# davidegraff/notorch

Measured on AMD Instinct MI355X. Metric: edge-messages/sec D-MPNN depth=3 h=300, QM9-shaped batches, 1/2/4/8 MI355X, higher is better.
Workload: dtype f32; 1 GPU; qm9-4096: 4096 qm9-shaped molecules per GPU, D-MPNN depth=3 hidden=300, ChempropBlock + Sum readout, reference collate (rev offset by nodes); molecules_per_gpu=4096, V_per_gpu=36362, E_per_gpu=77562, hidden=300, depth=3, parallelism=molecule-sharded x1, no collective on the forward path

## Files before the change

notorch_amd/csrc/update_fk.hip:

```cpp
#include <stdlib.h>

#include <atomic>

#include <type_traits>

#include "common.hpp"
#include "update.hpp"

#include "update_fk.hpp"

namespace nt {
int cu_count();
int xcd_count();
}

namespace nt {
namespace {
template <int RT, int CT, int ACT, int AACT, bool SUMONLY, int MAXL, bool DROP = false>
int launch_fk_t(const fk::Args& a, int grid, hipStream_t stream) {
  if constexpr (DROP)
    set_last_kernel(RT == 8 ? "update_fk_kernel: one 8-wave workgroup per CU, 128-row tiles, dropout in the epilogue"
                            : "update_fk_kernel: one 8-wave workgroup per CU, 64-row tiles, dropout in the epilogue");
  else
    set_last_kernel(RT == 8 ? "update_fk_kernel: one 8-wave workgroup per CU, 128-row tiles"
                            : "update_fk_kernel: one 8-wave workgroup per CU, 64-row tiles");
  fk::update_fk_kernel<RT, CT, ACT, AACT, SUMONLY, MAXL, 0, 8, DROP><<<grid, fk::kThreads, 0, stream>>>(a);
  NT_LAUNCH_CHECK();
  return NT_OK;
}

template <int CT, bool DROP = false>
int launch_fk_wide(const fk::Args& a, int maxl, int grid, hipStream_t stream) {
  [[maybe_unused]] const bool fused = a.SO != nullptr;
  const bool relu = a.act == NT_ACT_RELU;
  if constexpr (!DROP) {
    if (!fused) {
      if (relu) return launch_fk_t<8, CT, NT_ACT_RELU, NT_ACT_IDENTITY, true, 1>(a, grid, stream);
      if (a.act == NT_ACT_IDENTITY)
        return launch_fk_t<8, CT, NT_ACT_IDENTITY, NT_ACT_IDENTITY, true, 1>(a, grid, stream);
      return launch_fk_t<8, CT, -1, NT_ACT_IDENTITY, true, 1>(a, grid, stream);
    }
  }
  if (a.aact == NT_ACT_RELU)
    return maxl <= 3   ? launch_fk_t<8, CT, NT_ACT_RELU, NT_ACT_RELU, true, 3, DROP>(a, grid, stream)
           : maxl <= 8 ? launch_fk_t<8, CT, NT_ACT_RELU, NT_ACT_RELU, true, 8, DROP>(a, grid, stream)
                       : launch_fk_t<8, CT, NT_ACT_RELU, NT_ACT_RELU, true, 16, DROP>(a, grid, stream);
  return maxl <= 3   ? launch_fk_t<8, CT, NT_ACT_RELU, NT_ACT_IDENTITY, true, 3, DROP>(a, grid, stream)
         : maxl <= 8 ? launch_fk_t<8, CT, NT_ACT_RELU, NT_ACT_IDENTITY, true, 8, DROP>(a, grid, stream)
                     : launch_fk_t<8, CT, NT_ACT_RELU, NT_ACT_IDENTITY, true, 16, DROP>(a, grid, stream);
}

int fk_nw_env() {
  static const int v = [] {
    const char* e = getenv("NT_FK_NW");
    return e ? atoi(e) : 0;
  }();
  return v;
}
bool fk_nw4(int64_t h, bool fused, int act, int reduce, int aact) {
  return fk_nw_env() != 8 && fused && act == NT_ACT_RELU && reduce == NT_SUM &&
         (aact == NT_ACT_RELU || aact == NT_ACT_IDENTITY) && fk::nt_for(h) <= 20;
}
bool fk_nw4_forced() { return fk_nw_env() == 4; }

template <int AACT, int MAXL, bool DROP>
int launch_fk_nw4_t(const fk::Args& a, int grid, hipStream_t stream) {
  set_last_kernel(DROP ? "update_fk_kernel: two 4-wave workgroups per CU, 64-row tiles, dropout in the epilogue"
                       : "update_fk_kernel: two 4-wave workgroups per CU, 64-row tiles");
  fk::update_fk_kernel<4, 5, NT_ACT_RELU, AACT, true, MAXL, 0, 4, DROP><<<grid, 256, 0, stream>>>(a);
  NT_LAUNCH_CHECK();
  return NT_OK;
}

template <bool DROP = false>
int launch_fk_nw4(const fk::Args& a, int maxl, int grid, hipStream_t stream) {
  if (a.aact == NT_ACT_RELU)
    return maxl <= 3   ? launch_fk_nw4_t<NT_ACT_RELU, 3, DROP>(a, grid, stream)
           : maxl <= 8 ? launch_fk_nw4_t<NT_ACT_RELU, 8, DROP>(a, grid, stream)
                       : launch_fk_nw4_t<NT_ACT_RELU, 16, DROP>(a, grid, stream);
  return maxl <= 3   ? launch_fk_nw4_t<NT_ACT_IDENTITY, 3, DROP>(a, grid, stream)
         : maxl <= 8 ? launch_fk_nw4_t<NT_ACT_IDENTITY, 8, DROP>(a, grid, stream)
                     : launch_fk_nw4_t<NT_ACT_IDENTITY, 16, DROP>(a, grid, stream);
}

template <int CT, bool DROP = false>
int launch_fk_narrow(const fk::Args& a, int maxl, int grid, hipStream_t stream) {
  const bool fused = a.SO != nullptr;
  const bool relu = a.act == NT_ACT_RELU;
  const bool fast = !fused || (a.reduce == NT_SUM && (a.aact == NT_ACT_RELU || a.aact == NT_ACT_IDENTITY));
  if (fast) {
    if constexpr (!DROP) {
      if (!fused)
        return relu ? launch_fk_t<4, CT, NT_ACT_RELU, NT_ACT_IDENTITY, true, 1>(a, grid, stream)
                    : launch_fk_t<4, CT, -1, NT_ACT_IDENTITY, true, 1>(a, grid, stream);
    }
    if (a.aact == NT_ACT_RELU)
      return relu ? launch_fk_t<4, CT, NT_ACT_RELU, NT_ACT_RELU, true, 16, DROP>(a, grid, stream)
                  : launch_fk_t<4, CT, -1, NT_ACT_RELU, true, 16, DROP>(a, grid, stream);
    return relu ? launch_fk_t<4, CT, NT_ACT_RELU, NT_ACT_IDENTITY, true, 16, DROP>(a, grid, stream)
                : launch_fk_t<4, CT, -1, NT_ACT_IDENTITY, true, 16, DROP>(a, grid, stream);
  }
  (void)maxl;
  return launch_fk_t<4, CT, -1, -1, false, 16, DROP>(a, grid, stream);
}
}

int fk_tile_rows(int64_t h, int act, int reduce, int aact, bool fused) {
  if (fk_nw4_forced() && fk_nw4(h, fused, act, reduce, aact)) return 64;
  const bool wide_ok =
      !fused || (act == NT_ACT_RELU && reduce == NT_SUM && (aact == NT_ACT_RELU || aact == NT_ACT_IDENTITY));
  return (fk::nt_for(h) <= 24 && wide_ok) ? 128 : 64;
}

int launch_update_fk(const UpdateArgs& u, const void* Wimg, const float* amax_in, float* amax_out,
                     const int32_t* tile_ptr, int64_t ntiles, int tile_rows, int max_in_degree,
                     const void* row_table, int reduce, int aact, float aalpha, float* S_out,
                     const DropMask* drop) {
  const bool fused = tile_ptr != nullptr;
  NT_REQUIRE(fused == (S_out != nullptr), NT_EINVAL, "S_out must be given exactly with a tile plan");
  NT_REQUIRE(!fused || row_table, NT_EINVAL, "fp32 fused mode needs the row table (nt_dmpnn_row_table)");
  NT_REQUIRE(drop == nullptr || fused, NT_EUNSUPPORTED, "the dropout layer kernel needs a tile plan");
  NT_REQUIRE(amax_in != nullptr, NT_EINVAL, "fp32 update needs amax_in (max|H|, max|S| on the device)");
  NT_REQUIRE(u.h % 4 == 0, NT_EUNSUPPORTED, "fp32 update needs h % 4 == 0");
  NT_REQUIRE((u.E * u.h) / 4 < (int64_t(1) << 31) && (u.V * u.h) / 4 < (int64_t(1) << 31),
             NT_EUNSUPPORTED, "fp32 update: E*h and V*h must stay below 2^33");
  const int cap = fk_tile_rows(u.h, u.act, reduce, aact, fused);
  NT_REQUIRE(!fused || (tile_rows >= 1 && tile_rows <= cap), NT_EUNSUPPORTED,
             "tile plan rows exceed nt_dmpnn_fused_tile_rows for this layer");
  NT_REQUIRE(!fused || (max_in_degree >= 0 && max_in_degree <= 32), NT_EUNSUPPORTED,
             "fused aggregation needs max_in_degree <= 32");
  fk::Args a;
  a.H = u.H;
  a.S = u.S;
  a.src = u.src;
  a.rev = u.rev;
  a.Wimg = (const char*)Wimg;
  a.bias = u.b;
  a.amax_in = amax_in;
  a.amax_out = amax_out;
  a.V = u.V;
  a.E = u.E;
  a.h = (int)u.h;
  a.hv = (int)(u.h / 4);
  {
    const int64_t ldi = u.ldi ? u.ldi : u.h, ldo = u.ldo ? u.ldo : u.h;
    NT_REQUIRE(ldi >= u.h && ldo >= u.h && ldi % 4 == 0 && ldo % 4 == 0, NT_EINVAL,
               "row pitches must be >= h and multiples of 4");
    NT_REQUIRE((u.E * ldi) / 4 < (int64_t(1) << 31) && (u.V * ldi) / 4 < (int64_t(1) << 31) &&
                   (u.E * ldo) / 4 < (int64_t(1) << 31) && (u.V * ldo) / 4 < (int64_t(1) << 31),
               NT_EUNSUPPORTED, "fp32 update: E*ld and V*ld must stay below 2^33");
    a.ldiv = a.ldic = (int)(ldi / 4);
    a.ldoc = (int)(ldo / 4);
  }
  a.KS = fk::ks_for(u.h) < 4 ? 4 : (fk::ks_for(u.h) + 1) / 2 * 2;
  a.NT = fk::nt_for(u.h);
  a.residual = u.residual;
  a.act = u.act;
  a.alpha = u.alpha;
  a.tile_ptr = tile_ptr;
  a.rows = fused ? (const int4*)row_table : nullptr;
  a.reduce = reduce;
  a.aact = aact;
  a.aalpha = aalpha;
  a.O = u.H_out;
  a.SO = S_out;
  a.SP = u.S_part;
  if (drop) a.drop = *drop;
  a.nxcd = xcd_count();
  {
    static const int stagger = [] {
      const char* e = getenv("NT_FK_STAGGER");
      return e ? atoi(e) : 0;
    }();
    a.stagger = stagger;
  }
  a.ntiles = fused ? (int)ntiles : (int)((u.E + cap - 1) / cap);
  if (a.ntiles == 0) return NT_OK;
  const int grid = a.ntiles < cu_count() ? a.ntiles : cu_count();
  const int maxl = max_in_degree - 1;
  if (fused && tile_rows <= 64 && fk_nw4(u.h, true, u.act, reduce, aact)) {
    a.nchunks = 1;
    const int g4 = a.ntiles < 2 * cu_count() ? a.ntiles : 2 * cu_count();
    return drop ? launch_fk_nw4<true>(a, maxl, g4, u.stream) : launch_fk_nw4(a, maxl, g4, u.stream);
  }
  if (cap == 128) {
    a.nchunks = 1;
    return drop ? launch_fk_wide<3, true>(a, maxl, grid, u.stream) : launch_fk_wide<3>(a, maxl, grid, u.stream);
  }
  if (a.NT <= 24) {
    a.nchunks = 1;
    return drop ? launch_fk_narrow<3, true>(a, maxl, grid, u.stream) : launch_fk_narrow<3>(a, maxl, grid, u.stream);
  }
  a.nchunks = (a.NT + 31) / 32;
  return drop ? launch_fk_narrow<4, true>(a, maxl, grid, u.stream) : launch_fk_narrow<4>(a, maxl, grid, u.stream);
}

namespace {
template <int ACT, int AACT, bool SUMONLY, int MAXL>
int launch_fkb_t(const fk::Args& a, int grid, hipStream_t stream) {
  set_last_kernel("update_fk_kernel (bf16): one 8-wave workgroup per CU, 128-row tiles");
  fk::update_fk_kernel<8, 4, ACT, AACT, SUMONLY, MAXL, 1><<<grid, fk::kThreads, 0, stream>>>(a);
  NT_LAUNCH_CHECK();
  return NT_OK;
}
template <int AACT, int MAXL>
// ... 145 lines not shown
```

notorch_amd/csrc/update_fk.hpp:

```cpp
#pragma once

#include <type_traits>

#include "common.hpp"
#include "dropout.hpp"

namespace nt {
namespace fk {

typedef float f32x4 __attribute__((ext_vector_type(4)));
typedef _Float16 f16x8 __attribute__((ext_vector_type(8)));
typedef _Float16 f16x4 __attribute__((ext_vector_type(4)));
typedef __bf16 bf16x8 __attribute__((ext_vector_type(8)));
typedef __bf16 bf16x4 __attribute__((ext_vector_type(4)));

__device__ __forceinline__ float bf_lo(unsigned u) { return __uint_as_float(u << 16); }
__device__ __forceinline__ float bf_hi(unsigned u) { return __uint_as_float(u & 0xffff0000u); }
__device__ __forceinline__ float4 bf4_widen(uint4 v) {
  return float4{bf_lo(v.x), bf_hi(v.x), bf_lo(v.y), bf_hi(v.y)};
}
__device__ __forceinline__ uint2 bf4_pack(float a, float b, float c, float d) {
  const bf16x4 v = bf16x4{(__bf16)a, (__bf16)b, (__bf16)c, (__bf16)d};
  return __builtin_bit_cast(uint2, v);
}

constexpr int kThreads = 512;
constexpr int kWaves = 8;
constexpr int kImgHdr = 256;
constexpr int kEmaps = 4;
constexpr int kFlagStart = 1, kFlagEnd = 2, kFlagPart = 4;

__host__ __device__ constexpr int ks_for(int64_t h) { return (int)((h + 31) / 32); }
__host__ __device__ constexpr int nt_for(int64_t h) { return (int)((h + 15) / 16); }
__host__ __device__ constexpr int64_t image_bytes(int64_t h) {
  return kImgHdr + (int64_t)ks_for(h) * nt_for(h) * 2 * 1024;
}

struct Args {
  const float* H;
  const float* S;
  const int64_t* src;
  const int64_t* rev;
  const char* Wimg;
  const float* bias;
  const float* amax_in;
  float* amax_out;
  int64_t V, E;
  int h, hv, KS, NT, nchunks;
  int ldiv, ldic, ldoc;
  int residual, act;
  float alpha;
  const int* tile_ptr;
  int ntiles;
  const int4* rows;
  int reduce, aact;
  float aalpha;
  float* O;
  float* SO;
  float* SP = nullptr;
  int nxcd;
  int stagger;
  DropMask drop;
};

__host__ __device__ inline int scale_exp(float bound) {
  if (!(bound > 0.f) || !(bound <= 3.4028235e38f)) return 0;
  int e;
  frexpf(bound, &e);
  int s = 14 - e;
  return s > 24 ? 24 : s;
}

__device__ __forceinline__ float act_bound(float m, int act, float alpha) {
  if (act == NT_ACT_RELU || act == NT_ACT_IDENTITY) return m;
  const float a = fabsf(alpha) > 1.f ? fabsf(alpha) : 1.f;
  return a * m + a;
}

__device__ __forceinline__ void atomic_max_abs(float* p, float v) {
  atomic_max_nonneg(p, v);
}

__device__ __forceinline__ float wave_max(float v) {
#pragma unroll
  for (int o = 32; o >= 1; o >>= 1) v = fmaxf(v, __shfl_xor(v, o));
  return v;
}

__device__ __forceinline__ f16x8 as_f16x8(uint4 v) { return __builtin_bit_cast(f16x8, v); }

constexpr float kLoScale = 2048.f;
__device__ __forceinline__ _Float16 lo_part(float x, _Float16 x0) { return (_Float16)((x - (float)x0) * kLoScale); }

template <typename F, int... Is>
__device__ __forceinline__ void sfor_impl(F&& f, std::integer_sequence<int, Is...>) {
  (f(std::integral_constant<int, Is>{}), ...);
}
template <int N, typename F>
__device__ __forceinline__ void sfor(F&& f) {
  sfor_impl(f, std::make_integer_sequence<int, N>{});
}

__device__ __forceinline__ float dpp_shr1(float old, float x) {
  return __builtin_bit_cast(float, __builtin_amdgcn_update_dpp(__builtin_bit_cast(int, old),
                                                               __builtin_bit_cast(int, x), 0x111, 0xf,
                                                               0xf, false));
}
__device__ __forceinline__ float dpp_shr1_bc(float x) {
  return __builtin_bit_cast(float, __builtin_amdgcn_mov_dpp(__builtin_bit_cast(int, x), 0x111, 0xf, 0xf, true));
}
__device__ __forceinline__ float dpp_ror1(float x) {
  return __builtin_bit_cast(float, __builtin_amdgcn_update_dpp(0, __builtin_bit_cast(int, x), 0x121,
                                                               0xf, 0xf, false));
}

struct TileHead {
  int T, n;
};

template <int RT, bool PLAN>
__device__ __forceinline__ TileHead tile_head(const Args& a, int t) {
  if constexpr (PLAN) {
    const int T = a.tile_ptr[t], n = a.tile_ptr[t + 1] - T;
    return {T, n};
  }
  const int64_t T = (int64_t)t * (16 * RT);
  const int64_t n = a.E - T < 16 * RT ? a.E - T : 16 * RT;
  return {(int)T, (int)n};
}

template <int RT, bool FROM_ROWS>
__device__ __forceinline__ int4 row_raw(const Args& a, TileHead th, int row) {
  const int pos = th.T + (row < th.n ? row : 0);
  if constexpr (FROM_ROWS) return a.rows[pos];
  const int s = a.src ? (int)a.src[pos] : pos;
  const int q = a.rev ? (int)a.rev[pos] : -1;
  return int4{pos, s, q, kFlagStart | kFlagEnd};
}

__device__ __forceinline__ int2 row_offsets(const Args& a, int4 raw, bool valid) {
  const bool sok = valid && raw.y >= 0 && raw.y < a.V, qok = valid && raw.z >= 0 && raw.z < a.E;
  return int2{sok ? raw.y * a.ldiv : -1, qok ? raw.z * a.ldiv : -1};
}

__device__ __forceinline__ int4 row_entry(int4 raw, bool valid) {
  if (!valid) return int4{-1, -1, kFlagStart | kFlagEnd, 0};
  if (raw.w >= 0) return int4{raw.x, raw.w >> 2, raw.w & 3, 0};
  const int wv = -raw.w - 1;
  return int4{raw.x, wv >> 2, (wv & 3) | kFlagPart, 0};
}

constexpr int kGD = 2;

template <int RT, int CT, int PREC = 0, int NW = 8>
struct State {
  static constexpr int ROWS = 16 * RT;
  static constexpr int PPT = 2 * RT / NW;
  static constexpr int kPartB = RT * 1024;
  static constexpr int kBufB = 2 * kPartB;
  f32x4 acc[RT][CT];
  f32x4 bias[CT];
  uint4 wb[2][CT][2];
  f32x4 gs[kGD][PPT], gq[kGD][PPT];
  int gso[kGD], gqo[kGD];
  float mxH, mxS;
  int lane, wave, fr, g16, grt, grow, kp0, hv, hc, NT, CTC;
  int li, lo;
  float sA, sAW, inv;
  char* abuf;
  float* lbias;
  int4* emap;
  __amdgpu_buffer_rsrc_t wrsrc;
};

template <int RT, int CT, int ACT, int P, int PREC, int NW>
__device__ __forceinline__ void fk_gather(State<RT, CT, PREC, NW>& st, const Args& a, int soff, int qoff, int s) {
  st.gso[P] = soff;
  st.gqo[P] = qoff;
  const int sb = soff >= 0 ? soff : 0, qb = qoff >= 0 ? qoff : 0;
  const f32x4* S4 = reinterpret_cast<const f32x4*>(a.S);
  const f32x4* H4 = reinterpret_cast<const f32x4*>(a.H ? a.H : a.S);
  constexpr int NP = PREC ? 1 : State<RT, CT, PREC, NW>::PPT;
#pragma unroll
  for (int u = 0; u < NP; ++u) {
    int p = PREC ? 4 * s + st.g16 : 8 * s + st.kp0 + u;
    p = p < st.hv ? p : 0;
    st.gs[P][u] = S4[sb + p];
    st.gq[P][u] = H4[qb + p];
  }
}

template <int RT, int CT, int ACT, int P, int BUF, int PREC, int NW>
__device__ __forceinline__ void fk_split(State<RT, CT, PREC, NW>& st, const Args& a, int s) {
  using St = State<RT, CT, PREC, NW>;
  const bool sok = st.gso[P] >= 0, qok = st.gqo[P] >= 0;
  if constexpr (PREC == 1) {
    static_assert(RT == NW, "bf16 fk tiles: one row tile per wave");
    const bool in = 4 * s + st.g16 < st.hv;
    const uint4 su = __builtin_bit_cast(uint4, st.gs[P][0]), qu = __builtin_bit_cast(uint4, st.gq[P][0]);
    const unsigned sw[4] = {su.x, su.y, su.z, su.w}, qw[4] = {qu.x, qu.y, qu.z, qu.w};
    bf16x8 h0;
#pragma unroll
    for (int c = 0; c < 4; ++c) {
      const float q0 = act_t<ACT>(bf_lo(qw[c]), a.act, a.alpha), q1 = act_t<ACT>(bf_hi(qw[c]), a.act, a.alpha);
      h0[2 * c] = (__bf16)((sok && in ? bf_lo(sw[c]) : 0.f) - (qok && in ? q0 : 0.f));
      h0[2 * c + 1] = (__bf16)((sok && in ? bf_hi(sw[c]) : 0.f) - (qok && in ? q1 : 0.f));
    }
    *reinterpret_cast<bf16x8*>(st.abuf + BUF * St::kBufB + st.grt * 1024 + st.lane * 16) = h0;
    return;
  }
  float x[4 * St::PPT];
#pragma unroll
  for (int u = 0; u < St::PPT; ++u) {
    const bool in = 8 * s + st.kp0 + u < st.hv;
    const f32x4 sv = st.gs[P][u];
    const f32x4 qv = st.gq[P][u];
#pragma unroll
    for (int c = 0; c < 4; ++c) {
      const float q = act_t<ACT>(qv[c], a.act, a.alpha);
      const float av = (sok && in ? sv[c] : 0.f) - (qok && in ? q : 0.f);
      x[4 * u + c] = av * st.sA;
    }
  }
  char* base = st.abuf + BUF * St::kBufB + st.grt * 1024 + st.lane * 16 +
               (RT == NW ? 0 : 8 * (st.wave >> 2));
// ... 35 lines not shown
  }
}

__device__ __forceinline__ f16x8 w0_lo_scaled(uint4 w) {
  const unsigned k = 0x10001000u;
  uint4 r;
  asm volatile("v_pk_mul_f16 %0, %1, %2" : "=v"(r.x) : "v"(w.x), "s"(k));
  asm volatile("v_pk_mul_f16 %0, %1, %2" : "=v"(r.y) : "v"(w.y), "s"(k));
  asm volatile("v_pk_mul_f16 %0, %1, %2" : "=v"(r.z) : "v"(w.z), "s"(k));
  asm volatile("v_pk_mul_f16 %0, %1, %2" : "=v"(r.w) : "v"(w.w), "s"(k));
  return as_f16x8(r);
}

template <int PREC>
__device__ __forceinline__ f32x4 fk_mac(uint4 w0r, uint4 w1r, f16x8 a0, f16x8 a1, f32x4 t) {
  if constexpr (PREC == 1) {
    return __builtin_amdgcn_mfma_f32_16x16x32_bf16(__builtin_bit_cast(bf16x8, w0r), __builtin_bit_cast(bf16x8, a0),
                                                   t, 0, 0, 0);
  } else {
    const f16x8 w0 = as_f16x8(w0r), w1 = as_f16x8(w1r);
    t = __builtin_amdgcn_mfma_f32_16x16x32_f16(w1, a0, t, 0, 0, 0);
    t = __builtin_amdgcn_mfma_f32_16x16x32_f16(w0_lo_scaled(w0r), a1, t, 0, 0, 0);
    return __builtin_amdgcn_mfma_f32_16x16x32_f16(w0, a0, t, 0, 0, 0);
  }
}

template <int RT, int CT, int P, int PREC, int NW>
__device__ __forceinline__ void fk_mfma(State<RT, CT, PREC, NW>& st, int c, int nrt) {
  using St = State<RT, CT, PREC, NW>;
  const char* bb = st.abuf + P * St::kBufB + st.lane * 16;
  f16x8 a0 = *reinterpret_cast<const f16x8*>(bb);
  f16x8 a1 = PREC ? a0 : *reinterpret_cast<const f16x8*>(bb + St::kPartB);
#pragma unroll
  for (int rt = 0; rt < RT; ++rt) {
    if (rt < nrt) {
      f16x8 n0 = a0, n1 = a1;
      if (rt + 1 < RT) {
        n0 = *reinterpret_cast<const f16x8*>(bb + (rt + 1) * 1024);
        n1 = PREC ? n0 : *reinterpret_cast<const f16x8*>(bb + St::kPartB + (rt + 1) * 1024);
      }
#pragma unroll
      for (int j = 0; j < CT; ++j) {
        if (c * st.CTC + st.wave + NW * j < st.NT) {
          st.acc[rt][j] = fk_mac<PREC>(st.wb[P][j][0], st.wb[P][j][1], a0, a1, st.acc[rt][j]);
        }
      }
      a0 = n0;
      a1 = n1;
      __builtin_amdgcn_sched_barrier(0);
    }
  }
}

template <int RT, int CT, int PREC, int NW>
__device__ __forceinline__ void fk_resid_load(State<RT, CT, PREC, NW>& st, const Args& a, int i, int c, int j) {
  using St = State<RT, CT, PREC, NW>;
  int pc = 4 * (c * st.CTC + st.wave + NW * j) + st.g16;
  pc = pc < st.hc ? pc : 0;
#pragma unroll
  for (int rt = 0; rt < RT; ++rt) {
    const int e = st.emap[(i % kEmaps) * St::ROWS + 16 * rt + st.fr].x;
    const int64_t r = (int64_t)(e >= 0 ? e : 0) * st.li + pc;
    if constexpr (PREC == 1) {
      const uint2 v = reinterpret_cast<const uint2*>(a.H)[r];
      st.acc[rt][j] = __builtin_bit_cast(f32x4, uint4{v.x, v.y, 0u, 0u});
    } else {
      st.acc[rt][j] = reinterpret_cast<const f32x4*>(a.H)[r];
    }
  }
}

template <int RT, int CT, int PREC, int NW>
__device__ __forceinline__ void fk_bias_load(State<RT, CT, PREC, NW>& st, const Args& a, int c, int j) {
  int pc = 4 * (c * st.CTC + st.wave + NW * j) + st.g16;
  pc = (pc < st.hc && a.bias) ? pc : 0;
  if constexpr (PREC == 1) {
    const uint2 v = reinterpret_cast<const uint2*>(a.bias ? a.bias : a.S)[pc];
    st.bias[j] = __builtin_bit_cast(f32x4, uint4{v.x, v.y, 0u, 0u});
  } else {
    st.bias[j] = reinterpret_cast<const f32x4*>(a.bias ? a.bias : a.S)[pc];
  }
}

template <int RT, int CT, int PREC, int NW>
__device__ __forceinline__ void fk_resid_scale(State<RT, CT, PREC, NW>& st) {
  if constexpr (PREC == 1) {
#pragma unroll
    for (int rt = 0; rt < RT; ++rt)
#pragma unroll
      for (int j = 0; j < CT; ++j) {
        const float4 w = bf4_widen(__builtin_bit_cast(uint4, st.acc[rt][j]));
        st.acc[rt][j] = f32x4{w.x, w.y, w.z, w.w};
      }
    return;
  }
  const f32x4 s4 = f32x4{st.sAW, st.sAW, st.sAW, st.sAW};
#pragma unroll
  for (int rt = 0; rt < RT; ++rt)
#pragma unroll
    for (int j = 0; j < CT; ++j) st.acc[rt][j] = st.acc[rt][j] * s4;
}

constexpr bool fk_lds_bias(int NW) { return NW == 4; }

struct EpiCtx {
  const f32x4* b4;
  f32x4* O4;
  f32x4* SO4;
  const int4* em;
  int n;
  const f32x4* H4 = nullptr;
};

template <int RTI, int J, int RT, int CT, int AACT, bool SUMONLY, int MAXL, bool DROP, int PREC, int NW>
__device__ __forceinline__ void fk_epi_row(State<RT, CT, PREC, NW>& st, const Args& a, const EpiCtx& x0, int pc,
                                           bool pok, const f32x4& bj, f32x4& carry, float& ccnt) {
  if (16 * RTI < x0.n) {
    const int lo = st.lo;
    const int4 ri = x0.em[16 * RTI + st.fr];
    f32x4 o;
    [[maybe_unused]] f32x4 hres = f32x4{0.f, 0.f, 0.f, 0.f};
    if constexpr (DROP) {
      if (x0.H4) hres = x0.H4[(int64_t)(ri.x >= 0 ? ri.x : 0) * st.li + (pok ? pc : 0)];
    }
    uint2 ob = uint2{0u, 0u};
    if constexpr (PREC == 1) {
      ob = bf4_pack(st.acc[RTI][J][0] + bj[0], st.acc[RTI][J][1] + bj[1], st.acc[RTI][J][2] + bj[2],
                    st.acc[RTI][J][3] + bj[3]);
      const float4 w = bf4_widen(uint4{ob.x, ob.y, 0u, 0u});
      o = f32x4{w.x, w.y, w.z, w.w};
    } else {
#pragma unroll
      for (int q = 0; q < 4; ++q) o[q] = fmaf(st.acc[RTI][J][q], st.inv, bj[q]);
      if constexpr (DROP) {
        const uint64_t i0 = (uint64_t)(ri.x >= 0 ? ri.x : 0) * (uint64_t)a.h + (uint64_t)(4 * pc);
#pragma unroll
        for (int q = 0; q < 4; ++q) o[q] = hres[q] + drop_apply(a.drop, i0 + q, o[q]);
      }
    }
    const bool rok = ri.x >= 0 && pok;
    if (rok) {
      if constexpr (PREC == 1) {
        reinterpret_cast<uint2*>(x0.O4)[(int64_t)ri.x * lo + pc] = ob;
      } else {
        x0.O4[(int64_t)ri.x * lo + pc] = o;
        st.mxH = fmaxf(st.mxH, fmaxf(fmaxf(fabsf(o[0]), fabsf(o[1])), fmaxf(fabsf(o[2]), fabsf(o[3]))));
      }
    }
    if (x0.SO4 != nullptr) {
      const bool start = (ri.z & kFlagStart) != 0;
      f32x4 m;
#pragma unroll
      for (int q = 0; q < 4; ++q) m[q] = act_t<AACT>(o[q], a.aact, a.aalpha);
      f32x4 x = m, cin;
#pragma unroll
      for (int q = 0; q < 4; ++q) cin[q] = dpp_ror1(carry[q]);
      float cnt = 1.f;
      const float cinc = SUMONLY ? 0.f : dpp_ror1(ccnt);
#pragma unroll
      for (int it = 0; it < MAXL; ++it) {
        f32x4 y;
#pragma unroll
        for (int q = 0; q < 4; ++q) y[q] = dpp_shr1(cin[q], x[q]);
        if constexpr (SUMONLY) {
          x = start ? m : y + m;
        } else {
          const float yc = dpp_shr1(cinc, cnt);
          f32x4 z;
#pragma unroll
          for (int q = 0; q < 4; ++q) {
            const float mx = fmaxf(y[q], m[q]), mn = fminf(y[q], m[q]), sm = y[q] + m[q];
            z[q] = a.reduce == NT_MAX ? mx : (a.reduce == NT_MIN ? mn : sm);
          }
          x = start ? m : z;
          cnt = start ? 1.f : yc + 1.f;
        }
      }
      if ((ri.z & kFlagPart) && (ri.z & kFlagEnd) && rok) {
        if constexpr (PREC == 0) reinterpret_cast<f32x4*>(a.SP)[(int64_t)ri.y * st.hc + pc] = x;
      } else if ((ri.z & kFlagEnd) && rok) {
        f32x4 r = x;
        if (!SUMONLY && a.reduce == NT_MEAN) r = x / cnt;
        if constexpr (PREC == 1) {
          reinterpret_cast<uint2*>(x0.SO4)[(int64_t)ri.y * lo + pc] = bf4_pack(r[0], r[1], r[2], r[3]);
        } else {
          x0.SO4[(int64_t)ri.y * lo + pc] = r;
          st.mxS = fmaxf(st.mxS, fmaxf(fmaxf(fabsf(r[0]), fabsf(r[1])), fmaxf(fabsf(r[2]), fabsf(r[3]))));
        }
      }
      carry = x;
      ccnt = cnt;
    }
  }
  if constexpr (RTI + 1 < RT)
    fk_epi_row<RTI + 1, J, RT, CT, AACT, SUMONLY, MAXL, DROP>(st, a, x0, pc, pok, bj, carry, ccnt);
}

template <int J, int RT, int CT, int AACT, bool SUMONLY, int MAXL, bool DROP, int PREC, int NW>
__device__ __forceinline__ void fk_epi_col(State<RT, CT, PREC, NW>& st, const Args& a, const EpiCtx& x0, int i, int c,
                                           bool load_next, int i_next, int c_next) {
  const int ct = c * st.CTC + st.wave + NW * J;
  if (ct < st.NT) {
    const int pc = 4 * ct + st.g16;
    const bool pok = pc < st.hc;
    f32x4 bj = f32x4{0.f, 0.f, 0.f, 0.f};
    if constexpr (fk_lds_bias(NW)) {
      if (x0.b4 && pok) bj = *reinterpret_cast<const f32x4*>(st.lbias + 4 * pc);
    } else {
      if (x0.b4 && pok) bj = st.bias[J];
    }
    if constexpr (PREC == 1 && !fk_lds_bias(NW)) {
      const float4 w = bf4_widen(__builtin_bit_cast(uint4, bj));
      bj = f32x4{w.x, w.y, w.z, w.w};
    }
    f32x4 carry = f32x4{0.f, 0.f, 0.f, 0.f};
    float ccnt = 0.f;
    fk_epi_row<0, J, RT, CT, AACT, SUMONLY, MAXL, DROP>(st, a, x0, pc, pok, bj, carry, ccnt);
  }
  if (!fk_lds_bias(NW) && c_next != c) fk_bias_load(st, a, c_next, J);
  if (load_next) {
    fk_resid_load(st, a, i_next, c_next, J);
  } else {
#pragma unroll
    for (int rt = 0; rt < RT; ++rt) st.acc[rt][J] = f32x4{0.f, 0.f, 0.f, 0.f};
  }
  if constexpr (J + 1 < CT)
    fk_epi_col<J + 1, RT, CT, AACT, SUMONLY, MAXL, DROP>(st, a, x0, i, c, load_next, i_next, c_next);
}

template <int RT, int CT, int AACT, bool SUMONLY, int MAXL, bool DROP, int PREC, int NW>
__device__ __forceinline__ void fk_epilogue(State<RT, CT, PREC, NW>& st, const Args& a, int i, int c, int n,
                                            bool load_next, int i_next, int c_next) {
  EpiCtx x0;
  x0.b4 = reinterpret_cast<const f32x4*>(a.bias);
  x0.O4 = reinterpret_cast<f32x4*>(a.O);
  x0.SO4 = reinterpret_cast<f32x4*>(a.SO);
  x0.em = st.emap + (i % kEmaps) * State<RT, CT, PREC, NW>::ROWS;
  x0.n = n;
  if constexpr (DROP) {
    x0.H4 = (a.residual && a.H != nullptr) ? reinterpret_cast<const f32x4*>(a.H) : nullptr;
  }
  fk_epi_col<0, RT, CT, AACT, SUMONLY, MAXL, DROP>(st, a, x0, i, c, load_next, i_next, c_next);
}

constexpr int kLbiasB = 512 * 4;

__device__ __forceinline__ void fk_barrier() {
  __syncthreads();
}

template <int RT, int CT, int ACT, int AACT, bool SUMONLY, int MAXL, int PREC = 0, int NW = 8,
          bool DROP = false>
__global__ void __launch_bounds__(64 * NW, 2) update_fk_kernel(Args a) {
  static_assert(!DROP || PREC == 0, "the dropout epilogue is fp32 only (bf16: update_bf16_kernel)");
  constexpr bool FROM_ROWS = MAXL > 1;
  using St = State<RT, CT, PREC, NW>;
  constexpr int ROWS = St::ROWS;
  constexpr int kEmapB = kEmaps * ROWS * 16;
  static_assert(RT == NW || (RT == 4 && NW == 8), "row tiles per wave mapping");
  constexpr bool LB = fk_lds_bias(NW);
  constexpr int kExtraB = LB ? kLbiasB : 0;
  __shared__ __attribute__((aligned(16))) uint4 smem[(2 * St::kBufB + kEmapB + kExtraB) / 16];

  int t0 = (int)blockIdx.x, tstride = (int)gridDim.x, ntl;
  const int nx = a.nxcd;
  if (nx > 1 && (int)gridDim.x % nx == 0) {
    const int x = (int)blockIdx.x % nx, chunk = (a.ntiles + nx - 1) / nx;
    const int lo = x * chunk, hi = min(a.ntiles, lo + chunk);
    t0 = lo + (int)blockIdx.x / nx;
    tstride = (int)gridDim.x / nx;
    ntl = hi > t0 ? (hi - t0 + tstride - 1) / tstride : 0;
  } else {
    ntl = (a.ntiles - t0 + tstride - 1) / tstride;
  }
  if (ntl <= 0) return;
  auto tile = [&](int i) __attribute__((always_inline)) { return t0 + (i < ntl ? i : ntl - 1) * tstride; };
  if constexpr (NW == 4) {
    for (int q = (int)blockIdx.x >= (int)gridDim.x / 2 ? a.stagger : 0; q > 0; --q) __builtin_amdgcn_s_sleep(127);
  } else {
    for (int q = a.stagger * (((int)blockIdx.x / (nx > 0 ? nx : 1)) & 3); q > 0; --q) __builtin_amdgcn_s_sleep(127);
  }

  St st;
  const int tid = threadIdx.x;
  st.lane = tid & 63;
  st.wave = __builtin_amdgcn_readfirstlane(tid >> 6);
  st.fr = st.lane & 15;
  st.g16 = st.lane >> 4;
  st.grt = RT == NW ? st.wave : (st.wave & 3);
  st.grow = 16 * st.grt + st.fr;
  st.kp0 = RT == NW ? 2 * st.g16 : 2 * st.g16 + (st.wave >> 2);
  st.hv = a.hv;
  st.hc = a.h / 4;
  st.li = a.ldic;
  st.lo = a.ldoc;
  st.NT = a.NT;
  st.CTC = NW * CT;
  st.abuf = reinterpret_cast<char*>(smem);
  st.emap = reinterpret_cast<int4*>(st.abuf + 2 * St::kBufB);
  st.lbias = reinterpret_cast<float*>(st.abuf + 2 * St::kBufB + kEmapB);

  if constexpr (LB) {
    for (int q = tid; q < a.h; q += 64 * NW) {
      float b = 0.f;
      if (a.bias) {
        if constexpr (PREC == 1) b = __uint_as_float((unsigned)reinterpret_cast<const unsigned short*>(a.bias)[q] << 16);
        else b = a.bias[q];
      }
      st.lbias[q] = b;
    }
  }
  st.wrsrc = __builtin_amdgcn_make_buffer_rsrc(
      (void*)a.Wimg, (short)0, PREC ? ks_for(a.h) * nt_for(a.h) * 1024 : (int)image_bytes(a.h), 0x00020000);
  st.mxH = 0.f;
  st.mxS = 0.f;
  if constexpr (PREC == 1) {
    st.sA = st.sAW = st.inv = 1.f;
  } else {
    const float bound = a.src ? a.amax_in[1] + (a.rev ? act_bound(a.amax_in[0], a.act, a.alpha) : 0.f)
                              : a.amax_in[1];
    st.sA = ldexpf(1.f, scale_exp(bound));
    const float sW = *reinterpret_cast<const float*>(a.Wimg);
    st.sAW = st.sA * sW;
    st.inv = 1.f / st.sAW;
  }
  const bool resid = !DROP && a.residual && a.H != nullptr;
  const bool info_writer = st.g16 == 0 && st.wave < RT;
  const int SPT = a.nchunks * a.KS;

  int2 cur, nxt;
  int n_cur, n_nxt;
  int4 raw2;
  TileHead h2, h3;
  {
    const TileHead h0 = tile_head<RT, FROM_ROWS>(a, tile(0));
    const int4 r0 = row_raw<RT, FROM_ROWS>(a, h0, st.grow);
    const TileHead h1 = tile_head<RT, FROM_ROWS>(a, tile(1));
    const int4 r1 = row_raw<RT, FROM_ROWS>(a, h1, st.grow);
    h2 = tile_head<RT, FROM_ROWS>(a, tile(2));
    raw2 = row_raw<RT, FROM_ROWS>(a, h2, st.grow);
    h3 = tile_head<RT, FROM_ROWS>(a, tile(3));
    const bool v0 = st.grow < h0.n, v1 = st.grow < h1.n;
    cur = row_offsets(a, r0, v0);
    nxt = row_offsets(a, r1, v1);
    if (info_writer) {
      st.emap[0 * ROWS + st.grow] = row_entry(r0, v0);
      st.emap[1 * ROWS + st.grow] = row_entry(r1, v1);
    }
    n_cur = h0.n < ROWS ? h0.n : ROWS;
    n_nxt = h1.n < ROWS ? h1.n : ROWS;
  }
#pragma unroll
  for (int r = 0; r < RT; ++r)
#pragma unroll
    for (int j = 0; j < CT; ++j) st.acc[r][j] = f32x4{0.f, 0.f, 0.f, 0.f};

  __syncthreads();
  if (resid) {
#pragma unroll
    for (int j = 0; j < CT; ++j) fk_resid_load(st, a, 0, 0, j);
  }
#pragma unroll
  for (int j = 0; j < CT; ++j)
    if constexpr (!LB) fk_bias_load(st, a, 0, j);
  auto kcs = [&](int kk, int& cc, int& ss) __attribute__((always_inline)) {
    cc = kk / a.KS;
    ss = kk - cc * a.KS;
  };
  {
    int c1, s1;
    kcs(1, c1, s1);
    fk_gather<RT, CT, ACT, 0>(st, a, cur.x, cur.y, 0);
    fk_gather<RT, CT, ACT, 1>(st, a, cur.x, cur.y, 1 % a.KS);
    fk_load_w<RT, CT, 0>(st, 0, 0);
    fk_load_w<RT, CT, 1>(st, c1, s1);
    fk_split<RT, CT, ACT, 0, 0>(st, a, 0);
    fk_gather<RT, CT, ACT, 0>(st, a, cur.x, cur.y, 2 % a.KS);
  }
  fk_barrier();

  int i = 0, c = 0;
  const int U = ntl * a.nchunks;
  for (int u = 0; u < U; ++u) {
    fk_resid_scale(st);
    const int nrt = (n_cur + 15) >> 4;
    const int kb = c * a.KS;
    for (int s0 = 0; s0 < a.KS; s0 += 2) {
#pragma unroll
      for (int P = 0; P < 2; ++P) {
        const int k = kb + s0 + P;
        auto phase_mfma = [&]() __attribute__((always_inline)) {
          if (P == 0) fk_mfma<RT, CT, 0>(st, c, nrt);
          else fk_mfma<RT, CT, 1>(st, c, nrt);
          {
            int c2, s2;
            kcs(k + 2 < SPT ? k + 2 : k + 2 - SPT, c2, s2);
            if (P == 0) fk_load_w<RT, CT, 0>(st, c2, s2);
            else fk_load_w<RT, CT, 1>(st, c2, s2);
          }
        };
        auto phase_split = [&]() __attribute__((always_inline)) {
          const int k1 = k + 1 < SPT ? k + 1 : k + 1 - SPT;
          const int s1 = k1 - (k1 / a.KS) * a.KS;
          if (P == 0) fk_split<RT, CT, ACT, 1, 1>(st, a, s1);
          else fk_split<RT, CT, ACT, 0, 0>(st, a, s1);
          const int k3 = k + 3;
          const int adv = k3 >= SPT ? 1 : 0;
          const int s3 = (k3 - adv * SPT) % a.KS;
          const int so = adv == 0 ? cur.x : nxt.x, qo = adv == 0 ? cur.y : nxt.y;
          if (P == 0) fk_gather<RT, CT, ACT, 1>(st, a, so, qo, s3);
          else fk_gather<RT, CT, ACT, 0>(st, a, so, qo, s3);
        };
        phase_mfma();
        phase_split();
        fk_barrier();
      }
    }
    const bool last_c = c + 1 == a.nchunks;
    const int i_next = last_c ? (i + 1 < ntl ? i + 1 : i) : i, c_next = last_c ? 0 : c + 1;
    fk_epilogue<RT, CT, AACT, SUMONLY, MAXL, DROP>(st, a, i, c, n_cur, resid, i_next, c_next);
    c = c_next;
    if (last_c) {
      ++i;
      cur = nxt;
      n_cur = n_nxt;
      const bool v2 = st.grow < h2.n;
      nxt = row_offsets(a, raw2, v2);
      if (info_writer) st.emap[((i + 1) % kEmaps) * ROWS + st.grow] = row_entry(raw2, v2);
      n_nxt = h2.n < ROWS ? h2.n : ROWS;
      h2 = h3;
      raw2 = row_raw<RT, FROM_ROWS>(a, h2, st.grow);
      h3 = tile_head<RT, FROM_ROWS>(a, tile(i + 3));
    }
  }
  if (a.amax_out) {
    const float mh = wave_max(st.mxH), ms = wave_max(st.mxS);
    __shared__ float amx[2][NW];
    if (st.lane == 0) {
      amx[0][st.wave] = mh;
      amx[1][st.wave] = ms;
    }
    __syncthreads();
    if (tid == 0) {
      float bh = amx[0][0], bs = amx[1][0];
#pragma unroll
      for (int w = 1; w < NW; ++w) {
        bh = fmaxf(bh, amx[0][w]);
        bs = fmaxf(bs, amx[1][w]);
      }
      atomic_max_abs(a.amax_out, bh);
      if (a.SO) atomic_max_abs(a.amax_out + 1, bs);
    }
  }
}

__global__ void __launch_bounds__(256) row_table_kernel(const int32_t* __restrict__ perm,
                                                        const int32_t* __restrict__ dsts,
                                                        const int64_t* __restrict__ src,
                                                        const int64_t* __restrict__ rev, int64_t V,
                                                        int64_t E, int4* __restrict__ out) {
  for (int64_t p = blockIdx.x * 256LL + threadIdx.x; p < E; p += (int64_t)gridDim.x * 256) {
    const int e = perm[p];
    const int64_t s = src[e], q = rev[e];
    const int v = dsts[p];
    const bool start = p == 0 || dsts[p - 1] != v, end = p + 1 == E || dsts[p + 1] != v;
    out[p] = int4{e, (s >= 0 && s < V) ? (int)s : -1, (q >= 0 && q < E) ? (int)q : -1,
                  (v << 2) | (start ? kFlagStart : 0) | (end ? kFlagEnd : 0)};
  }
}

constexpr int kScaleParts = 32;
__global__ void __launch_bounds__(256) pack_fk_scale_kernel(const float* __restrict__ W, int64_t h,
                                                            int64_t w_stride, int64_t img_stride,
                                                            char* __restrict__ img) {
  const float* Wl = W + blockIdx.y * w_stride;
  const int64_t n = h * h, per = (n + kScaleParts - 1) / kScaleParts;
  const int64_t lo = blockIdx.x * per, hi = lo + per < n ? lo + per : n;
  __shared__ float red[4];
  float m = 0.f;
  for (int64_t q = lo + threadIdx.x; q < hi; q += 256) m = fmaxf(m, fabsf(Wl[q]));
  m = wave_max(m);
  if ((threadIdx.x & 63) == 0) red[threadIdx.x >> 6] = m;
  __syncthreads();
  if (threadIdx.x == 0)
    reinterpret_cast<float*>(img + blockIdx.y * img_stride)[1 + blockIdx.x] =
        fmaxf(fmaxf(red[0], red[1]), fmaxf(red[2], red[3]));
}

__global__ void __launch_bounds__(256) pack_fk_kernel(const float* __restrict__ W, int64_t h, int KS,
                                                      int NT, int64_t w_stride, int64_t img_stride,
                                                      char* __restrict__ img) {
  const int layer = blockIdx.y;
  const float* Wl = W + layer * w_stride;
  char* out = img + layer * img_stride;
  float mw = 0.f;
#pragma unroll
  for (int i = 1; i <= kScaleParts; ++i) mw = fmaxf(mw, reinterpret_cast<const float*>(out)[i]);
  const float sW = ldexpf(1.f, scale_exp(mw));
  if (blockIdx.x == 0 && threadIdx.x == 0) *reinterpret_cast<float*>(out) = sW;
  const int64_t slots = (int64_t)KS * NT * 2 * 64;
  const int64_t q = blockIdx.x * 256LL + threadIdx.x;
  if (q >= slots) return;
  const int l = (int)(q & 63);
  const int64_t blk = q >> 6;
// ... 96 lines not shown
```

Measured before the change: 598.0 million edge-messages/s.

## Add 32-bit byte-offset epilogue with buffer resource residual loads and ballot masks

Adds a B32 epilogue path for fp32 sum-only kernels without dropout. The row map stores precomputed 32-bit byte offsets, residual loads go through a buffer resource, and start/end/hub flags become wave ballot bitmasks that drive the segmented scan and masked stores. The amax reduction switches to LDS atomics. The aim is to cut 64-bit address arithmetic, per-row flag decoding and VGPR pressure in the epilogue. A 64-bit fallback is chosen automatically for large tensors or via an env var, which adds a template variant and code complexity.

```diff
diff --git a/notorch_amd/csrc/update_fk.hip b/notorch_amd/csrc/update_fk.hip
--- a/notorch_amd/csrc/update_fk.hip
+++ b/notorch_amd/csrc/update_fk.hip
@@ -24,7 +24,11 @@
   else
     set_last_kernel(RT == 8 ? "update_fk_kernel: one 8-wave workgroup per CU, 128-row tiles"
                             : "update_fk_kernel: one 8-wave workgroup per CU, 64-row tiles");
-  fk::update_fk_kernel<RT, CT, ACT, AACT, SUMONLY, MAXL, 0, 8, DROP><<<grid, fk::kThreads, 0, stream>>>(a);
+  constexpr bool A64 = !DROP && SUMONLY && ACT >= 0;
+  if (A64 && a.addr64)
+    fk::update_fk_kernel<RT, CT, ACT, AACT, SUMONLY, MAXL, 0, 8, DROP, A64><<<grid, fk::kThreads, 0, stream>>>(a);
+  else
+    fk::update_fk_kernel<RT, CT, ACT, AACT, SUMONLY, MAXL, 0, 8, DROP><<<grid, fk::kThreads, 0, stream>>>(a);
   NT_LAUNCH_CHECK();
   return NT_OK;
 }
@@ -67,7 +71,10 @@
 int launch_fk_nw4_t(const fk::Args& a, int grid, hipStream_t stream) {
   set_last_kernel(DROP ? "update_fk_kernel: two 4-wave workgroups per CU, 64-row tiles, dropout in the epilogue"
                        : "update_fk_kernel: two 4-wave workgroups per CU, 64-row tiles");
-  fk::update_fk_kernel<4, 5, NT_ACT_RELU, AACT, true, MAXL, 0, 4, DROP><<<grid, 256, 0, stream>>>(a);
+  if (!DROP && a.addr64)
+    fk::update_fk_kernel<4, 5, NT_ACT_RELU, AACT, true, MAXL, 0, 4, DROP, !DROP><<<grid, 256, 0, stream>>>(a);
+  else
+    fk::update_fk_kernel<4, 5, NT_ACT_RELU, AACT, true, MAXL, 0, 4, DROP><<<grid, 256, 0, stream>>>(a);
   NT_LAUNCH_CHECK();
   return NT_OK;
 }
@@ -151,6 +158,12 @@
                NT_EUNSUPPORTED, "fp32 update: E*ld and V*ld must stay below 2^33");
     a.ldiv = a.ldic = (int)(ldi / 4);
     a.ldoc = (int)(ldo / 4);
+    static const bool force64 = [] {
+      const char* e = getenv("NT_FK_ADDR64");
+      return e && atoi(e) != 0;
+    }();
+    const int64_t rows = u.E > u.V ? u.E : u.V, ld = ldi > ldo ? ldi : ldo;
+    a.addr64 = force64 || rows * ld * 4 >= (int64_t(1) << 31);
   }
   a.KS = fk::ks_for(u.h) < 4 ? 4 : (fk::ks_for(u.h) + 1) / 2 * 2;
   a.NT = fk::nt_for(u.h);
diff --git a/notorch_amd/csrc/update_fk.hpp b/notorch_amd/csrc/update_fk.hpp
--- a/notorch_amd/csrc/update_fk.hpp
+++ b/notorch_amd/csrc/update_fk.hpp
@@ -60,6 +60,7 @@
   float* SP = nullptr;
   int nxcd;
   int stagger;
+  int addr64 = 0;
   DropMask drop;
 };
 
@@ -112,6 +113,16 @@
 __device__ __forceinline__ float dpp_ror1(float x) {
   return __builtin_bit_cast(float, __builtin_amdgcn_update_dpp(0, __builtin_bit_cast(int, x), 0x121,
                                                                0xf, 0xf, false));
+}
+__device__ __forceinline__ float dpp_ror1_bc(float x) {
+  return __builtin_bit_cast(float, __builtin_amdgcn_mov_dpp(__builtin_bit_cast(int, x), 0x121, 0xf, 0xf, true));
+}
+
+__device__ __forceinline__ float amax4(float m, f32x4 v) {
+  float r;
+  asm("v_max3_f32 %0, %1, |%2|, |%3|" : "=v"(r) : "v"(m), "v"(v[0]), "v"(v[1]));
+  asm("v_max3_f32 %0, %1, |%2|, |%3|" : "=v"(m) : "v"(r), "v"(v[2]), "v"(v[3]));
+  return m;
 }
 
 struct TileHead {
@@ -143,11 +154,22 @@
   return int2{sok ? raw.y * a.ldiv : -1, qok ? raw.z * a.ldiv : -1};
 }
 
-__device__ __forceinline__ int4 row_entry(int4 raw, bool valid) {
-  if (!valid) return int4{-1, -1, kFlagStart | kFlagEnd, 0};
-  if (raw.w >= 0) return int4{raw.x, raw.w >> 2, raw.w & 3, 0};
-  const int wv = -raw.w - 1;
-  return int4{raw.x, wv >> 2, (wv & 3) | kFlagPart, 0};
+constexpr unsigned kOobOff = 0x80000000u;
+
+template <bool B32>
+__device__ __forceinline__ int4 row_entry(int4 raw, bool valid, unsigned lo, unsigned li) {
+  if constexpr (B32) {
+    if (!valid) return int4{(int)kOobOff, (int)kOobOff, kFlagStart | kFlagEnd, (int)kOobOff};
+    const int wv = raw.w >= 0 ? raw.w : -raw.w - 1;
+    const int oo = (int)((unsigned)raw.x * lo * 16u), ho = (int)((unsigned)raw.x * li * 16u);
+    const int so = raw.w >= 0 ? (int)((unsigned)(wv >> 2) * lo * 16u) : wv >> 2;
+    return int4{oo, so, (wv & 3) | (raw.w >= 0 ? 0 : kFlagPart), ho};
+  } else {
+    if (!valid) return int4{-1, -1, kFlagStart | kFlagEnd, 0};
+    if (raw.w >= 0) return int4{raw.x, raw.w >> 2, raw.w & 3, 0};
+    const int wv = -raw.w - 1;
+    return int4{raw.x, wv >> 2, (wv & 3) | kFlagPart, 0};
+  }
 }
 
 constexpr int kGD = 2;
@@ -171,6 +193,7 @@
   float* lbias;
   int4* emap;
   __amdgpu_buffer_rsrc_t wrsrc;
+  __amdgpu_buffer_rsrc_t hrsrc;
 };
 
 template <int RT, int CT, int ACT, int P, int PREC, int NW>
@@ -312,9 +335,18 @@
   }
 }
 
-template <int RT, int CT, int PREC, int NW>
+template <bool B32, int RT, int CT, int PREC, int NW>
 __device__ __forceinline__ void fk_resid_load(State<RT, CT, PREC, NW>& st, const Args& a, int i, int c, int j) {
   using St = State<RT, CT, PREC, NW>;
+  if constexpr (B32) {
+    const int cb = __builtin_amdgcn_readfirstlane(64 * (c * st.CTC + st.wave + NW * j));
+#pragma unroll
+    for (int rt = 0; rt < RT; ++rt) {
+      const unsigned off = (unsigned)st.emap[(i % kEmaps) * St::ROWS + 16 * rt + st.fr].w + 16u * st.g16;
+      st.acc[rt][j] = __builtin_bit_cast(f32x4, __builtin_amdgcn_raw_buffer_load_b128(st.hrsrc, off, cb, 0));
+    }
+    return;
+  }
   int pc = 4 * (c * st.CTC + st.wave + NW * j) + st.g16;
   pc = pc < st.hc ? pc : 0;
 #pragma unroll
@@ -363,6 +395,12 @@
 
 constexpr bool fk_lds_bias(int NW) { return NW == 4; }
 
+__device__ __forceinline__ uint64_t rows_mask(unsigned m16) {
+  const unsigned m = m16 * 0x10001u;
+  return (uint64_t)m << 32 | m;
+}
+
+template <int RT>
 struct EpiCtx {
   const f32x4* b4;
   f32x4* O4;
@@ -370,12 +408,72 @@
   const int4* em;
   int n;
   const f32x4* H4 = nullptr;
+  unsigned sk[RT / 2], ek[RT / 2], hk[RT / 2];
+  int cb;
 };
 
-template <int RTI, int J, int RT, int CT, int AACT, bool SUMONLY, int MAXL, bool DROP, int PREC, int NW>
-__device__ __forceinline__ void fk_epi_row(State<RT, CT, PREC, NW>& st, const Args& a, const EpiCtx& x0, int pc,
-                                           bool pok, const f32x4& bj, f32x4& carry, float& ccnt) {
-  if (16 * RTI < x0.n) {
+template <int AACT, int MAXL, bool FIRST>
+__device__ __forceinline__ void fk_scan(const Args& a, const f32x4& o, bool startp, bool inj, f32x4& carry, f32x4& x) {
+  f32x4 m;
+#pragma unroll
+  for (int q = 0; q < 4; ++q) {
+    if constexpr (AACT == NT_ACT_RELU) asm("v_max_f32 %0, 0, %1" : "=v"(m[q]) : "v"(o[q]));
+    else m[q] = act_t<AACT>(o[q], a.aact, a.aalpha);
+  }
+  if constexpr (!FIRST) {
+#pragma unroll
+    for (int q = 0; q < 4; ++q) {
+      float t = dpp_ror1_bc(carry[q]) + m[q];
+      asm("" : "+v"(t));
+      m[q] = inj ? t : m[q];
+    }
+  }
+  x = m;
+#pragma unroll
+  for (int it = 0; it < MAXL; ++it) {
+#pragma unroll
+    for (int q = 0; q < 4; ++q) {
+      const float z = dpp_shr1_bc(x[q]) + m[q];
+      x[q] = startp ? m[q] : z;
+    }
+  }
+  carry = x;
+}
+
+template <int RTI, int J, bool B32, int RT, int CT, int AACT, bool SUMONLY, int MAXL, bool DROP, int PREC, int NW>
+__device__ __forceinline__ void fk_epi_row(State<RT, CT, PREC, NW>& st, const Args& a, const EpiCtx<RT>& x0, int pc,
+                                           bool pok, uint64_t pokm, const f32x4& bj, f32x4& carry, float& ccnt) {
+  if constexpr (B32) {
+    if (16 * RTI < x0.n) {
+      const unsigned v16 = x0.n - 16 * RTI >= 16 ? 0xffffu : (1u << (x0.n - 16 * RTI)) - 1u;
+      const uint64_t vm = rows_mask(v16) & pokm;
+      const int2 ro = *reinterpret_cast<const int2*>(&x0.em[16 * RTI + st.fr]);
+      const unsigned g = 16u * (unsigned)st.g16 + (unsigned)x0.cb + 64u * NW * J;
+      f32x4 o;
+#pragma unroll
+      for (int q = 0; q < 4; ++q) o[q] = fmaf(st.acc[RTI][J][q], st.inv, bj[q]);
+      if (__builtin_amdgcn_inverse_ballot_w64(vm)) {
+        *reinterpret_cast<f32x4*>(reinterpret_cast<char*>(a.O) + ((unsigned)ro.x + g)) = o;
+        st.mxH = amax4(st.mxH, o);
+      }
+      if constexpr (MAXL > 1) {
+        f32x4 x;
+        constexpr int SH = 16 * (RTI & 1);
+        const unsigned sk = x0.sk[RTI / 2] >> SH & 0xffffu;
+        fk_scan<AACT, MAXL, RTI == 0>(a, o, __builtin_amdgcn_inverse_ballot_w64(rows_mask(sk | 1u)),
+                                      __builtin_amdgcn_inverse_ballot_w64(rows_mask(~sk & 1u)), carry, x);
+        if (__builtin_amdgcn_inverse_ballot_w64(rows_mask(x0.ek[RTI / 2] >> SH & 0xffffu) & vm)) {
+          *reinterpret_cast<f32x4*>(reinterpret_cast<char*>(a.SO) + ((unsigned)ro.y + g)) = x;
+          st.mxS = amax4(st.mxS, x);
+        }
+        if ((x0.hk[RTI / 2] >> SH & 0xffffu) != 0) {
+          if (__builtin_amdgcn_inverse_ballot_w64(rows_mask(x0.hk[RTI / 2] >> SH & 0xffffu) & vm))
+            *reinterpret_cast<f32x4*>(reinterpret_cast<char*>(a.SP) +
+                                      ((unsigned)ro.y * (16u * (unsigned)st.hc) + g)) = x;
+        }
+      }
+    }
+  } else if (16 * RTI < x0.n) {
     const int lo = st.lo;
     const int4 ri = x0.em[16 * RTI + st.fr];
     f32x4 o;
@@ -453,19 +551,19 @@
     }
   }
   if constexpr (RTI + 1 < RT)
-    fk_epi_row<RTI + 1, J, RT, CT, AACT, SUMONLY, MAXL, DROP>(st, a, x0, pc, pok, bj, carry, ccnt);
-}
-
-template <int J, int RT, int CT, int AACT, bool SUMONLY, int MAXL, bool DROP, int PREC, int NW>
-__device__ __forceinline__ void fk_epi_col(State<RT, CT, PREC, NW>& st, const Args& a, const EpiCtx& x0, int i, int c,
-                                           bool load_next, int i_next, int c_next) {
+    fk_epi_row<RTI + 1, J, B32, RT, CT, AACT, SUMONLY, MAXL, DROP>(st, a, x0, pc, pok, pokm, bj, carry, ccnt);
+}
+
+template <int J, bool B32, int RT, int CT, int AACT, bool SUMONLY, int MAXL, bool DROP, int PREC, int NW>
+__device__ __forceinline__ void fk_epi_col(State<RT, CT, PREC, NW>& st, const Args& a, const EpiCtx<RT>& x0, int i,
+                                           int c, bool load_next, int i_next, int c_next) {
   const int ct = c * st.CTC + st.wave + NW * J;
   if (ct < st.NT) {
     const int pc = 4 * ct + st.g16;
     const bool pok = pc < st.hc;
     f32x4 bj = f32x4{0.f, 0.f, 0.f, 0.f};
     if constexpr (fk_lds_bias(NW)) {
-      if (x0.b4 && pok) bj = *reinterpret_cast<const f32x4*>(st.lbias + 4 * pc);
+      if (B32 || (x0.b4 && pok)) bj = *reinterpret_cast<const f32x4*>(st.lbias + 4 * pc);
     } else {
       if (x0.b4 && pok) bj = st.bias[J];
     }
@@ -475,23 +573,25 @@
     }
     f32x4 carry = f32x4{0.f, 0.f, 0.f, 0.f};
     float ccnt = 0.f;
-    fk_epi_row<0, J, RT, CT, AACT, SUMONLY, MAXL, DROP>(st, a, x0, pc, pok, bj, carry, ccnt);
+    const uint64_t pokm = __builtin_amdgcn_ballot_w64(pok);
+    fk_epi_row<0, J, B32, RT, CT, AACT, SUMONLY, MAXL, DROP>(st, a, x0, pc, pok, pokm, bj, carry, ccnt);
   }
   if (!fk_lds_bias(NW) && c_next != c) fk_bias_load(st, a, c_next, J);
-  if (load_next) {
-    fk_resid_load(st, a, i_next, c_next, J);
+  if (B32 || load_next) {
+    fk_resid_load<B32>(st, a, i_next, c_next, J);
   } else {
 #pragma unroll
     for (int rt = 0; rt < RT; ++rt) st.acc[rt][J] = f32x4{0.f, 0.f, 0.f, 0.f};
   }
   if constexpr (J + 1 < CT)
-    fk_epi_col<J + 1, RT, CT, AACT, SUMONLY, MAXL, DROP>(st, a, x0, i, c, load_next, i_next, c_next);
-}
-
-template <int RT, int CT, int AACT, bool SUMONLY, int MAXL, bool DROP, int PREC, int NW>
+    fk_epi_col<J + 1, B32, RT, CT, AACT, SUMONLY, MAXL, DROP>(st, a, x0, i, c, load_next, i_next, c_next);
+}
+
+template <bool B32, int RT, int CT, int AACT, bool SUMONLY, int MAXL, bool DROP, int PREC, int NW>
 __device__ __forceinline__ void fk_epilogue(State<RT, CT, PREC, NW>& st, const Args& a, int i, int c, int n,
                                             bool load_next, int i_next, int c_next) {
-  EpiCtx x0;
+  static_assert(!B32 || (PREC == 0 && !DROP && SUMONLY), "the 32-bit epilogue: fp32 sums without dropout");
+  EpiCtx<RT> x0;
   x0.b4 = reinterpret_cast<const f32x4*>(a.bias);
   x0.O4 = reinterpret_cast<f32x4*>(a.O);
   x0.SO4 = reinterpret_cast<f32x4*>(a.SO);
@@ -500,7 +600,23 @@
   if constexpr (DROP) {
     x0.H4 = (a.residual && a.H != nullptr) ? reinterpret_cast<const f32x4*>(a.H) : nullptr;
   }
-  fk_epi_col<0, RT, CT, AACT, SUMONLY, MAXL, DROP>(st, a, x0, i, c, load_next, i_next, c_next);
+  if constexpr (B32) {
+    x0.cb = __builtin_amdgcn_readfirstlane(64 * (c * st.CTC + st.wave));
+  }
+  if constexpr (B32 && MAXL > 1) {
+#pragma unroll
+    for (int r2 = 0; r2 < RT / 2; ++r2) x0.sk[r2] = x0.ek[r2] = x0.hk[r2] = 0u;
+#pragma unroll
+    for (int rt = 0; rt < RT; ++rt) {
+      const int zf = x0.em[16 * rt + st.fr].z;
+      const bool hub = (zf & kFlagPart) != 0, end = (zf & kFlagEnd) != 0;
+      const int sh = 16 * (rt & 1);
+      x0.sk[rt / 2] |= ((unsigned)__builtin_amdgcn_ballot_w64((zf & kFlagStart) != 0) & 0xffffu) << sh;
+      x0.ek[rt / 2] |= ((unsigned)__builtin_amdgcn_ballot_w64(end && !hub) & 0xffffu) << sh;
+      x0.hk[rt / 2] |= ((unsigned)__builtin_amdgcn_ballot_w64(end && hub) & 0xffffu) << sh;
+    }
+  }
+  fk_epi_col<0, B32, RT, CT, AACT, SUMONLY, MAXL, DROP>(st, a, x0, i, c, load_next, i_next, c_next);
 }
 
 constexpr int kLbiasB = 512 * 4;
@@ -510,7 +626,7 @@
 }
 
 template <int RT, int CT, int ACT, int AACT, bool SUMONLY, int MAXL, int PREC = 0, int NW = 8,
-          bool DROP = false>
+          bool DROP = false, bool A64 = false>
 __global__ void __launch_bounds__(64 * NW, 2) update_fk_kernel(Args a) {
   static_assert(!DROP || PREC == 0, "the dropout epilogue is fp32 only (bf16: update_bf16_kernel)");
   constexpr bool FROM_ROWS = MAXL > 1;
@@ -572,6 +688,10 @@
   }
   st.wrsrc = __builtin_amdgcn_make_buffer_rsrc(
       (void*)a.Wimg, (short)0, PREC ? ks_for(a.h) * nt_for(a.h) * 1024 : (int)image_bytes(a.h), 0x00020000);
+  constexpr bool B32 = PREC == 0 && !DROP && !A64 && SUMONLY && ACT >= 0;
+  if constexpr (B32)
+    st.hrsrc = __builtin_amdgcn_make_buffer_rsrc((void*)a.H, (short)0,
+                                                 a.residual && a.H ? (int)(a.E * a.ldic * 16) : 0, 0x00020000);
   st.mxH = 0.f;
   st.mxS = 0.f;
   if constexpr (PREC == 1) {
@@ -604,8 +724,8 @@
     cur = row_offsets(a, r0, v0);
     nxt = row_offsets(a, r1, v1);
     if (info_writer) {
-      st.emap[0 * ROWS + st.grow] = row_entry(r0, v0);
-      st.emap[1 * ROWS + st.grow] = row_entry(r1, v1);
+      st.emap[0 * ROWS + st.grow] = row_entry<B32>(r0, v0, st.lo, st.li);
+      st.emap[1 * ROWS + st.grow] = row_entry<B32>(r1, v1, st.lo, st.li);
     }
     n_cur = h0.n < ROWS ? h0.n : ROWS;
     n_nxt = h1.n < ROWS ? h1.n : ROWS;
@@ -615,10 +735,12 @@
 #pragma unroll
     for (int j = 0; j < CT; ++j) st.acc[r][j] = f32x4{0.f, 0.f, 0.f, 0.f};
 
+  __shared__ unsigned amx[2];
+  if (B32 && tid < 2) amx[tid] = 0u;
   __syncthreads();
   if (resid) {
 #pragma unroll
-    for (int j = 0; j < CT; ++j) fk_resid_load(st, a, 0, 0, j);
+    for (int j = 0; j < CT; ++j) fk_resid_load<B32>(st, a, 0, 0, j);
   }
 #pragma unroll
   for (int j = 0; j < CT; ++j)
@@ -678,7 +800,7 @@
     }
     const bool last_c = c + 1 == a.nchunks;
     const int i_next = last_c ? (i + 1 < ntl ? i + 1 : i) : i, c_next = last_c ? 0 : c + 1;
-    fk_epilogue<RT, CT, AACT, SUMONLY, MAXL, DROP>(st, a, i, c, n_cur, resid, i_next, c_next);
+    fk_epilogue<B32, RT, CT, AACT, SUMONLY, MAXL, DROP>(st, a, i, c, n_cur, resid, i_next, c_next);
     c = c_next;
     if (last_c) {
       ++i;
@@ -686,30 +808,40 @@
       n_cur = n_nxt;
       const bool v2 = st.grow < h2.n;
       nxt = row_offsets(a, raw2, v2);
-      if (info_writer) st.emap[((i + 1) % kEmaps) * ROWS + st.grow] = row_entry(raw2, v2);
+      if (info_writer) st.emap[((i + 1) % kEmaps) * ROWS + st.grow] = row_entry<B32>(raw2, v2, st.lo, st.li);
       n_nxt = h2.n < ROWS ? h2.n : ROWS;
       h2 = h3;
       raw2 = row_raw<RT, FROM_ROWS>(a, h2, st.grow);
       h3 = tile_head<RT, FROM_ROWS>(a, tile(i + 3));
     }
   }
-  if (a.amax_out) {
-    const float mh = wave_max(st.mxH), ms = wave_max(st.mxS);
-    __shared__ float amx[2][NW];
-    if (st.lane == 0) {
-      amx[0][st.wave] = mh;
-      amx[1][st.wave] = ms;
-    }
+  if constexpr (!B32) {
+    if (a.amax_out) {
+      const float mh = wave_max(st.mxH), ms = wave_max(st.mxS);
+      __shared__ float amw[2][NW];
+      if (st.lane == 0) {
+        amw[0][st.wave] = mh;
+        amw[1][st.wave] = ms;
+      }
+      __syncthreads();
+      if (tid == 0) {
+        float bh = amw[0][0], bs = amw[1][0];
+#pragma unroll
+        for (int w = 1; w < NW; ++w) {
+          bh = fmaxf(bh, amw[0][w]);
+          bs = fmaxf(bs, amw[1][w]);
+        }
+        atomic_max_abs(a.amax_out, bh);
+        if (a.SO) atomic_max_abs(a.amax_out + 1, bs);
+      }
+    }
+  } else if (a.amax_out) {
+    atomicMax(&amx[0], __float_as_uint(st.mxH));
+    atomicMax(&amx[1], __float_as_uint(st.mxS));
     __syncthreads();
     if (tid == 0) {
-      float bh = amx[0][0], bs = amx[1][0];
-#pragma unroll
-      for (int w = 1; w < NW; ++w) {
-        bh = fmaxf(bh, amx[0][w]);
-        bs = fmaxf(bs, amx[1][w]);
-      }
-      atomic_max_abs(a.amax_out, bh);
-      if (a.SO) atomic_max_abs(a.amax_out + 1, bs);
+      atomic_max_abs(a.amax_out, __uint_as_float(amx[0]));
+      if (a.SO) atomic_max_abs(a.amax_out + 1, __uint_as_float(amx[1]));
     }
   }
 }
```

After: 602.2 million edge-messages/s (median of 4 runs). Within noise of the previous version (+0.7%).
